# tangtang888/video-edge-ai-proxy

Measured on AMD Instinct MI355X. Metric: decoded FPS (whole node) + p50 VideoLatestImage latency, 256×1080p RTSP, higher is better.
Workload: dtype uint8 (BGR24 frames; bf16-capable consumer path)

## Files before the change

csrc/bind_ext.h:

```cpp
#pragma once
#include <pybind11/pybind11.h>

void bind_net(pybind11::module_& m);
void bind_mux(pybind11::module_& m);
void bind_hevc(pybind11::module_& m);
void bind_bus(pybind11::module_& m);
void bind_rpc(pybind11::module_& m);
void bind_dbk(pybind11::module_& m);
void bind_hevc_lf(pybind11::module_& m);
```

csrc/bindings.cpp:

```cpp
#include <malloc.h>

#include <pybind11/numpy.h>
#include <pybind11/pybind11.h>
#include <pybind11/stl.h>

#include "vep/hostprof.h"
#include "vep/avc.h"
#include "vep/avc_cavlc.h"
#include "vep/avc_recon.h"
#include "vep/bench_driver.h"
#include "vep/cabac.h"
#include "vep/codec.h"
#include "vep/gpu.h"
#include "vep/h264.h"
#include "vep/hevc_ctu.h"
#include "vep/hevc_dec.h"
#include "vep/hevc_kern.h"
#include "vep/jpeg.h"
#include "vep/scale.h"
#include "bind_ext.h"
#include "vep/runtime.h"
#include "vep/synth.h"

namespace py = pybind11;
// ... 2401 lines not shown
  m.def("letterbox_geometry", [](int src_w, int src_h, int size, bool even) {
    gpu::LetterboxDesc d{};
    d.src_w = src_w;
    d.src_h = src_h;
    gpu::fill_letterbox_geometry(d, size, even);
    return py::make_tuple(d.nw, d.nh, d.pad_x, d.pad_y);
  }, py::arg("src_w"), py::arg("src_h"), py::arg("size"), py::arg("even") = false);

  bind_net(m);
  bind_mux(m);
  bind_hevc(m);
  bind_bus(m);
  bind_rpc(m);
  bind_dbk(m);
  bind_hevc_lf(m);
}
```

csrc/vep/avc.cpp:

```cpp
#include "avc.h"

#include <immintrin.h>

#include <algorithm>
#include <array>

#include "avc_cavlc.h"
#include "avc_internal.h"
#include "fanout.h"

namespace vep::avc {

using h264::Pps;
using h264::Sps;


void MbNeighbours::reset(int wmbs, int hmbs, bool ring) {
  w_ = wmbs;
  h_ = hmbs;
  cur_ = -1;
  run_slice_ = ~0u;
  run_start_ = 0;
  announced_ = 0;
  const size_t n = size_t(wmbs) * hmbs;
// ... 1434 lines not shown
        }
        pair_.have |= u8(1 << int(sh.bottom_field));
        pair_.poc[int(sh.bottom_field)] = pic->poc;
      } else {
        pic->target = pick_slot();
      }
      if (sh.nal_ref_idc != 0 && sps.profile_idc != 66) {
        col_built = col_pool_->acquire([](ColMotion&) {});
        col_built->wmbs = W;
        col_built->hmbs = Hp;
        col_built->corners = sps.direct_8x8;
        col_built->b.resize(size_t(W) * Hp * size_t(sps.direct_8x8 ? 4 : 16));
        colb.col = col_built.get();
        pic->colb = &colb;
      }
      got = true;
    } else {
      VEP_CHECK(&sps == act_sps, "slices of one picture reference different SPSs");
      if (sh.field_pic != first.field_pic || sh.bottom_field != first.bottom_field) {
        VEP_CHECK(next_nal != nullptr, "H.264: one access unit holds several pictures");
        *next_nal = i;
        break;
      }
      if (sh.type() == h264::kB || pic->info.pict_type == 'I') pic->info.pict_type = "PBISi"[sh.type()];
    }
    if (sh.field_pic) build_field_lists(sh, sps, pic->poc);
    else build_lists(sh, sps, pic->poc);
    std::array<std::vector<u32>, 2> uids;
    for (int l = 0; l < 2; ++l)
      for (const auto& e : list_[l]) uids[size_t(l)].push_back(e.uid);
// ... 128 lines not shown
  } else {
    if (first.nal_ref_idc != 0) {
      mark_references(first, *act_sps, pic->target, pic->poc, uid, std::move(col_built));
    }
    const bool boundary = first.idr() || first.has_mmco5();
    if (first.has_mmco5()) pic->poc = 0;
    bump(*pic, out_of(*pic), boundary, boundary && (hard_flush || reorder_cur_ == 0));
  }
  if (missing || par) validate(*pic);
  else validate_picture(*pic);
  return pic;
}

Decoder::Decoder() {
  if (const char* e = std::getenv("VEP_AVC_SLICE_THREADS")) parallel_slices_ = e[0] != '0';
}
Decoder::~Decoder() = default;

void Decoder::parse_slice_data(MbNeighbours& nb, Picture& pic, const SliceHdr& sh, const Sps& sps, const Pps& pps,
                               const u8* data, size_t n, size_t bitpos, int slice_idx,
                               const std::vector<ListEntry> (&lists)[2]) {
  if (legacy_slice(sh, sps, pps)) {
    Bits br(data, n, bitpos);
    const size_t stop = BitReader(data, n).stop_bit_pos();
    SliceCtx sc{sh, pps, slice_idx, sh.type() == h264::kP, sh.qp, lists[0]};
    const int total = pic.nmbs();
    int mb = sh.first_mb;
    VEP_CHECK(mb < total, "first_mb_in_slice past end of picture");
    bool more = true;
    while (more) {
// ... 15 lines not shown
      more = br.pos() < stop;
      ++mb;
    }
    return;
  }
  SliceEnv env;
  env.sh = &sh;
  env.sps = &sps;
  env.pps = &pps;
  env.slice = slice_idx;
  env.list[0] = &lists[0];
  env.list[1] = &lists[1];
  env.cur_poc = pic.poc;
  env.scaling = h264::resolve_scaling(sps, pps);
  env.field = sh.field_pic;
  decode_slice_generic(nb, pic, env, data, n, bitpos);
}

static inline void validate_mb(const Picture& p, const MbRec& m, bool written = false) {
  const size_t ncoef = p.coefs.size(), nmv = p.mvs.size();
  VEP_CHECK(m.kind <= kI8x8, "macroblock kind out of range");
  VEP_CHECK(p.cf == 2 || m.chroma_coded < 0x100, "chroma block mask out of range");
  VEP_CHECK(m.qp <= 51 + p.qp_bias && m.qpc <= 51 + p.qpc_bias && m.qpc2 <= 51 + p.qpc_bias,
            "macroblock QP out of range");
  if (m.kind == kIPcm) {
    const size_t ns = p.cf == 2 ? size_t(kPcmMaxSamples) : size_t(kPcmMbBytes);
    VEP_CHECK(size_t(m.coef) + (p.bd > 8 ? ns : ns / 2) <= ncoef, "I_PCM samples outside the pool");
    return;
  }
  const size_t nw = size_t(coef_words(m));
// ... 354 lines not shown
  const __m256i tl = _mm256_setr_epi32(0, 0, 2, 2, 0, 0, 2, 2);
  const u32 all = u32(_mm256_movemask_epi8(_mm256_and_si256(_mm256_cmpeq_epi32(a, v0), _mm256_cmpeq_epi32(b, v0))));
  const u32 q8 = u32(_mm256_movemask_epi8(_mm256_and_si256(_mm256_cmpeq_epi32(a, _mm256_permutevar8x32_epi32(a, tl)),
                                                           _mm256_cmpeq_epi32(b, _mm256_permutevar8x32_epi32(b, tl)))));
  return (all == 0xFFFFFFFFu ? 1u : 0u) | (q8 == 0xFFFFFFFFu ? 2u : 0u);
#else
  u32 v[16];
  std::memcpy(v, mv, sizeof v);
  bool u16 = true, u8x8 = true;
  for (int b = 1; b < 16; ++b) u16 &= v[b] == v[0];
  for (int b = 0; b < 16; ++b) u8x8 &= v[b] == v[((b >> 3) << 3) | (b & 2)];
  return (u16 ? 1u : 0u) | (u8x8 ? 2u : 0u);
#endif
}

static inline void store_motion(Picture& pic, MbRec& m, const MbState& s) {
  const int nl = (m.flags & kMbL1) ? 2 : 1;
  u32 u = 3;
  for (int l = 0; l < nl; ++l) u &= motion_uniformity(&s.mv[l][0][0]);
  m.flags |= (u & 1) ? kMbMv16 : ((u & 2) ? kMbMv8x8 : 0);
  m.mv = u32(pic.mvs.size());
  const int per = (u & 1) ? 2 : ((u & 2) ? 8 : 32);
  i16* out = pic.mvs.extend(size_t(per * nl));
  for (int l = 0; l < nl; ++l, out += per) {
    const i16* v = &s.mv[l][0][0];
    if (per == 2) {
      std::memcpy(out, v, 4);
    } else if (per == 8) {
      std::memcpy(out, v, 4);
      std::memcpy(out + 2, v + 4, 4);
      std::memcpy(out + 4, v + 16, 4);
      std::memcpy(out + 6, v + 20, 4);
    } else {
      std::memcpy(out, v, 64);
// ... 15 lines not shown
  store_motion(pic, m, s);
  ++pic.inter_mbs;
  if (!(m.dbk & 1)) pic.deblock = true;
  for (int k = 0; k < 4; ++k) {
    const int r0 = m.ref[k], r1 = m.ref1[k];
    VEP_CHECK((r0 != 0xFF || r1 != 0xFF) && (r0 == 0xFF || r0 < pic.dpb_slots) && (r1 == 0xFF || r1 < pic.dpb_slots) &&
                  (r1 == 0xFF || (m.flags & kMbL1)),
              "skipped macroblock reference slot outside the DPB");
  }
  VEP_CHECK(m.qp <= 51 + pic.qp_bias && m.qpc <= 51 + pic.qpc_bias && m.qpc2 <= 51 + pic.qpc_bias,
            "macroblock QP out of range");
  store_rec(&pic.mbs[size_t(mb)], m);
  if (pic.colb) pic.colb->store(mb, s);
}

void store_mb(Picture& pic, int mb, MbRec m, const MbState& s, const MbResidual* res, const u8* pcm,
              const WpEntry* wp) {
  m.coef = u32(pic.coefs.size());
  m.luma_coded = 0;
  m.chroma_coded = 0;
  if (m.kind == kIPcm) {
    VEP_CHECK(pcm, "I_PCM macroblock without samples");
    const size_t ns = pic.cf == 2 ? size_t(kPcmMaxSamples) : size_t(kPcmMbBytes);
    const size_t o = pic.coefs.size(), nb = pic.bd > 8 ? 2 * ns : ns;
    pic.coefs.resize(o + nb / 2);
    std::memcpy(pic.coefs.data() + o, pcm, nb);
  } else if (res && (res->luma | res->chroma)) {
    m.luma_coded = res->luma;
    m.chroma_coded = res->chroma;
    if (res->t8) m.flags |= kMbT8x8;
    const i16* grp[32];
    int ng = 0;
// ... 10 lines not shown
    for (int g = 0; g < ng; ++g) {
      mask[g] = nonzero_mask16(grp[g]);
      nv += __builtin_popcount(mask[g]);
    }
    const size_t o = pic.coefs.size();
    i16* out = pic.coefs.extend(size_t(ng + nv) + 8);
    std::memcpy(out, mask, size_t(ng) * sizeof(u16));
    i16* v = out + ng;
    for (int g = 0; g < ng; ++g) v = compact16(grp[g], mask[g], v);
    pic.coefs.resize(o + size_t(ng + nv));
  }
  m.mv = 0;
  m.wp = 0;
  m.flags &= u8(~(kMbMv8x8 | kMbMv16));
  if (m.kind == kSkip || m.kind == kInter) {
    store_motion(pic, m, s);
    if (wp && (m.flags & kMbWp)) {
      m.wp = u32(pic.wps.size());
      pic.wps.insert(pic.wps.end(), wp, wp + 4);
    } else {
      m.flags &= u8(~kMbWp);
    }
    ++pic.inter_mbs;
  } else if (m.kind == kIPcm) {
    ++pic.inter_mbs;
  } else {
    ++pic.intra_mbs;
  }
  m.res = is_intra(m.kind) && m.kind != kIPcm && (m.luma_coded | m.chroma_coded) ? u32(pic.intra_res++) : kNoRes;
  if (!(m.dbk & 1)) pic.deblock = true;
  validate_written_mb(pic, m);
// ... 356 lines not shown
```

csrc/vep/avc.h:

```cpp
#pragma once

#include <array>
#include <map>
#include <memory>

#include "hostmem.h"
#include "recycle.h"
#include "avc_recon.h"
#include "codec.h"

namespace vep::avc {

constexpr int kMaxDpbSlots = 34;

struct AuMeta {
  i64 pts = 0, dts = 0, arrival_ms = 0;
  i64 tag = 0;
  bool keyframe = false, corrupt = false;
};

struct OutFrame {
  int slot = -1;
  PictureInfo info;
  AuMeta au;
// ... 71 lines not shown

struct MbState {
  u8 kind = 0xFF;
  u8 skip = 0;
  u8 direct16 = 0;
  u8 direct8 = 0;
  u8 t8x8 = 0;
  u8 cbp = 0;
  u8 chroma_mode = 0;
  u8 qp = 0;
  u16 slice = 0;
  u16 cbf = 0;
  u8 cbf_dc = 0;
  u8 cbf_cac[2] = {0, 0};
  i8 ref[2][4] = {{-1, -1, -1, -1}, {-1, -1, -1, -1}};
  i16 mv[2][16][2] = {};
  u8 mvd[2][16][2] = {};
  u8 tc[16] = {};
  u8 tcc[2][8] = {};
  u8 i4[16] = {};
};

class MbNeighbours {
 public:
  void reset(int wmbs, int hmbs, bool ring = false);
  void begin(int mb);
  MbState& at(int mb) { return st_[size_t(mb) & mask_]; }
  const MbState& at(int mb) const { return st_[size_t(mb) & mask_]; }
  int wmbs() const { return w_; }
  int hmbs() const { return h_; }
  int mb_at(int mb, int x, int y) const;
  bool mb_available(int mb, int nb) const {
    const size_t i = size_t(nb) & mask_;
    return nb >= 0 && stamp_[size_t(nb)] == epoch_ && tag_[i] == u32(nb) && st_[i].kind != 0xFF &&
           st_[i].slice == st_[size_t(mb) & mask_].slice;
// ... 320 lines not shown
  bool field_mode_ = false;
  struct OpenPair {
    bool open = false;
    int slot = -1, frame_num = 0, bottom = 0;
    int poc[2] = {0, 0};
    bool ref = false, boundary = false, hard = false;
    u8 have = 0;
    OutFrame f;
  } pair_;
  void close_pair(Picture& pic);

 public:
  Decoder();
  ~Decoder();
  u64 parallel_slices_run() const { return parallel_slices_run_; }
  u64 mmco_ops[7] = {0, 0, 0, 0, 0, 0, 0};
  u64 list_mods = 0, long_term_marked = 0;
  u64 redundant_slices_skipped = 0;
};

void cpu_reconstruct(const Picture& pic, std::vector<HostSurface>& slots);
void weave_fields(const HostSurface& top, const HostSurface& bottom, HostSurface& frame);

struct MbLevels {
  int luma[16][16];
  int dc[16];
  int cdc[2][4];
  int cac[2][4][16];
  u16 lmask = 0;
  u8 cmask = 0;
// ... 9 lines not shown
      for (int b = 0; b < 4; ++b) {
        if (cdc[c][b]) dcmask |= u8(2 << c);
        for (int k = 0; k < 16; ++k)
          if (cac[c][b][k]) cmask |= u8(1u << (c * 4 + b));
      }
  }
};
struct MbResidual {
  i16 blk[32][16];
  i16 b8[4][64];
  u16 luma = 0;
  u16 chroma = 0;
  bool t8 = false;
};
void dequantize_mb(const MbLevels& lv, bool i16x16, int qp, int qpc, MbResidual& out);
void store_mb(Picture& pic, int mb, MbRec m, const MbState& s, const MbResidual* res, const u8* pcm,
              const WpEntry* wp = nullptr);
void store_skip_mb(Picture& pic, int mb, MbRec& m, const MbState& s);
void cpu_reconstruct_mb(const Picture& pic, int mb, std::vector<HostSurface>& slots);
void cpu_deblock(const Picture& pic, HostSurface& target);
void intra4x4_neighbours(const Picture& pic, int mb, int idx, const HostSurface& T, Intra4Nb& n);
void intra16_neighbours(const Picture& pic, int mb, const HostSurface& T, Intra16Nb& n);
void chroma_neighbours(const Picture& pic, int mb, int c, const HostSurface& T, IntraChromaNb& n);
void intra8x8_neighbours(const Picture& pic, int mb, int q, const HostSurface& T, int* f, bool& has_top,
                         bool& has_left);

class StreamEncoder {
 public:
  virtual ~StreamEncoder() = default;
  virtual std::shared_ptr<AccessUnit> next() = 0;
  virtual const HostSurface& reconstruction() const = 0;
  virtual const HostSurface& source() const = 0;
  virtual i64 last_pts() const = 0;
// ... 93 lines not shown
```

csrc/vep/avc_internal.h:

```cpp
#pragma once

#include <array>

#include "avc.h"
#include "bits.h"

namespace vep::avc {

struct SliceEnv {
  const SliceHdr* sh = nullptr;
  const h264::Sps* sps = nullptr;
  const h264::Pps* pps = nullptr;
  int slice = 0;
  const std::vector<ListEntry>* list[2] = {nullptr, nullptr};
  int cur_poc = 0;
  h264::ScalingLists scaling;
  bool field = false;
};

void decode_slice_generic(MbNeighbours& nb, Picture& pic, const SliceEnv& env, const u8* data, size_t n,
                          size_t bitpos);

WpEntry wp_entry(const SliceEnv& env, int r0, int r1);

std::shared_ptr<ColMotion> build_col_motion(const MbNeighbours& nb, int wmbs, int hmbs,
                                            const std::vector<std::array<std::vector<u32>, 2>>& slice_uids,
                                            bool corners, Recycler<ColMotion>* pool = nullptr);

void predict_inter(const std::vector<HostSurface>& slots, const MbRec& m, const i16* mv0, const i16* mv1,
                   const WpEntry* wp, int mx, int my, int* py, int (*pc)[128], int structure = 0);

struct MbDesc {
// ... 54 lines not shown
```

csrc/vep/avc_mb.cpp:

```cpp
#include <algorithm>
#include <memory>
#include <cstddef>
#include <cstring>

#include "avc_cabac.h"
#include "avc_cavlc.h"
#include "avc_internal.h"

namespace vep::avc {

namespace {

struct Dequant {
  int ls4[6][6][16];
  int ls8[2][6][64];
  explicit Dequant(const h264::ScalingLists& sl) {
    for (int l = 0; l < 6; ++l)
      for (int m = 0; m < 6; ++m)
        for (int k = 0; k < 16; ++k) {
          const int pos = kZigzag4x4[k];
          ls4[l][m][pos] = int(sl.l4[l][k]) * norm_adjust(m, pos >> 2, pos & 3);
        }
    for (int l = 0; l < 2; ++l)
      for (int m = 0; m < 6; ++m)
// ... 48 lines not shown
    cf_ = sps_.chroma_format_idc;
    nbc_ = cf_ == 2 ? 8 : 4;
    weighted_ = (type_ == h264::kP && pps_.weighted_pred) || (type_ == h264::kB && pps_.weighted_bipred_idc != 0);
    implicit_ = type_ == h264::kB && pps_.weighted_bipred_idc == 2;
    for (int l = 0; l < 2; ++l) {
      std::fill(std::begin(slot_[l]), std::end(slot_[l]), u8(0xFF));
      if (const auto* lst = env_.list[l])
        for (size_t k = 0; k < lst->size() && k + 1 < std::size(slot_[l]); ++k)
          if ((*lst)[k].slot >= 0) slot_[l][k + 1] = u8((*lst)[k].slot);
    }
    for (int q = 0; q < 52 + qpbd_ && q < int(std::size(qpc_tab_[0])); ++q) {
      qpc_tab_[0][q] = u8(chroma_qp_bd(q - qpbd_, pps_.chroma_qp_index_offset, qpbdc_) + qpbdc_);
      qpc_tab_[1][q] = u8(chroma_qp_bd(q - qpbd_, pps_.second_chroma_qp_index_offset, qpbdc_) + qpbdc_);
    }
    fast_direct_ = !kWrite && type_ == h264::kB && sh_.direct_spatial && sps_.direct_8x8 && !weighted_;
  }

  Bits* br = nullptr;
  BitWriter* bw = nullptr;
  Bins* bins = nullptr;
  cabac::Decoder* cabac = nullptr;
  cabac::Encoder* cenc = nullptr;
  const MbDesc* want = nullptr;
  int prev_qpd_nz = 0;

  int qp() const { return qp_; }

  int ue(u32 v) {
    if constexpr (kWrite) {
      bw->ue(v);
      return int(v);
// ... 9 lines not shown
      return br->se();
    }
  }
  int u(int n, u32 v) {
    if constexpr (kWrite) {
      bw->u(n, v);
      return int(v);
    } else {
      return int(br->u(n));
    }
  }

  static void clear_but_mv(MbState& s) {
    static const MbState z{};
    std::memcpy(static_cast<void*>(&s), &z, offsetof(MbState, mv));
    std::memcpy(static_cast<void*>(&s.mvd), &z.mvd, sizeof(MbState) - offsetof(MbState, mvd));
  }

  bool read_skip_flag(int mb, bool v = false) {
    MbState& s = nb_.at(mb);
    if constexpr (kWrite) s = MbState{};
    else clear_but_mv(s);
    s.slice = u16(env_.slice);
    nb_.begin(mb);
    auto cond = [&](int m) { return m >= 0 && !nb_.at(m).skip ? 1 : 0; };
    const int inc = cond(nb_.mb_at(mb, -1, 0)) + cond(nb_.mb_at(mb, 0, -1));
    return bins->mb_skip(type_ == h264::kB, inc, v) != 0;
  }

  void skip_mb(int mb, bool fresh) {
    MbState& s = nb_.at(mb);
    if (fresh) {
      s = MbState{};
      s.slice = u16(env_.slice);
      nb_.begin(mb);
    }
    s.kind = kSkip;
    s.skip = 1;
    s.qp = u8(qp_ + qpbd_);
    MbResidual res;
    res.luma = 0;
    res.chroma = 0;
    if (type_ == h264::kP) {
      s.ref[0][0] = s.ref[0][1] = s.ref[0][2] = s.ref[0][3] = 0;
      need_ref(0, 0);
      int mv[2];
      nb_.pskip_mv(mb, mv);
      for (auto& v : s.mv[0]) {
        v[0] = i16(mv[0]);
        v[1] = i16(mv[1]);
      }
    } else {
      s.direct16 = 1;
      s.direct8 = 0xF;
      if (fast_direct_) direct16_spatial(mb, s);
      else direct(mb, s, 0xF);
    }
    prev_qpd_nz = 0;
    if (!weighted_ && !kWrite) emit_skip(mb, s);
    else emit(mb, s, res, 0, 0, nullptr);
  }

  void coded_mb(int mb, bool fresh) {
    MbState& s = nb_.at(mb);
    if (fresh) {
      s = MbState{};
      s.slice = u16(env_.slice);
      nb_.begin(mb);
    } else if constexpr (!kWrite) {
      std::memset(static_cast<void*>(s.mv), 0, sizeof s.mv);
    }
    int mbt = read_mb_type(mb, kWrite ? want->mb_type : 0);
    int itype = -1;
    if (type_ == h264::kI) {
      itype = mbt;
    } else if (type_ == h264::kP) {
      VEP_CHECK(mbt <= 30, "bad P mb_type");
      if (mbt >= 5) itype = mbt - 5;
    } else {
      VEP_CHECK(mbt <= 48, "bad B mb_type");
      if (mbt >= 23) itype = mbt - 23;
    }
    VEP_CHECK(itype <= 25, "bad intra mb_type");
    MbResidual res;
    res.luma = 0;
    res.chroma = 0;
// ... 26 lines not shown
    if (s.kind == kInter && (cbp & 15) && pps_.transform_8x8_mode && no_small &&
        !(type_ == h264::kB && mbt == 0 && !sps_.direct_8x8))
      s.t8x8 = u8(read_t8x8(mb, kWrite && want->t8x8));
    int qp = qp_;
    if ((cbp & 15) || (cbp >> 4) || s.kind == kI16x16) {
      const int dqp = read_qp_delta(kWrite ? want->qp_delta : 0);
      VEP_CHECK(dqp >= -(26 + qpbd_ / 2) && dqp <= 25 + qpbd_ / 2, "mb_qp_delta out of range");
      qp = (qp + dqp + 52 + 2 * qpbd_) % (52 + qpbd_) - qpbd_;
      prev_qpd_nz = dqp != 0;
    } else {
      prev_qpd_nz = 0;
    }
    qp_ = qp;
    s.qp = u8(qp + qpbd_);
    residual(mb, s, res, cbp & 15, cbp >> 4, qp + qpbd_, intra);
    emit(mb, s, res, i16_mode, s.chroma_mode, nullptr);
  }

  void skip_motion(int mb, MbState& out) {
    MbState& s = nb_.at(mb);
    s = MbState{};
    s.slice = u16(env_.slice);
    nb_.begin(mb);
    out = MbState{};
    out.slice = s.slice;
    if (type_ == h264::kP) {
      for (int k = 0; k < 4; ++k) out.ref[0][k] = 0;
      int mv[2];
      nb_.pskip_mv(mb, mv);
      for (auto& v : out.mv[0]) {
        v[0] = i16(mv[0]);
// ... 282 lines not shown
  }
  static void set_mv(MbState& s, int list, const Part& p, int mx, int my) {
    VEP_CHECK(mx >= -32768 && mx <= 32767 && my >= -32768 && my <= 32767, "motion vector out of range");
    for (int y = p.y4; y < p.y4 + p.h4; ++y)
      for (int x = p.x4; x < p.x4 + p.w4; ++x) {
        s.mv[list][y * 4 + x][0] = i16(mx);
        s.mv[list][y * 4 + x][1] = i16(my);
      }
  }

  bool inter_pred(int mb, MbState& s, int mbt) {
    const bool b = type_ == h264::kB;
    if (b && mbt == 0) {
      s.direct16 = 1;
      s.direct8 = 0xF;
      if (fast_direct_) direct16_spatial(mb, s);
      else direct(mb, s, 0xF);
      return true;
    }
    if ((!b && mbt <= 2) || (b && mbt <= 21)) {
      Part parts[2];
      int np;
      u8 pred[2];
      int shape;
      if (!b) {
        shape = mbt;
        pred[0] = pred[1] = 1;
      } else {
        shape = mbt <= 3 ? 0 : ((mbt & 1) ? 2 : 1);
        pred[0] = kBPart[mbt][0];
        pred[1] = kBPart[mbt][1];
      }
      np = shape == 0 ? 1 : 2;
      for (int i = 0; i < np; ++i) {
        if (shape == 0) parts[i] = {0, 0, 4, 4, 0};
        else if (shape == 1) parts[i] = {0, 2 * i, 4, 2, 1};
        else parts[i] = {2 * i, 0, 2, 4, 2};
      }
      int refs[2][2] = {{-1, -1}, {-1, -1}};
      for (int l = 0; l < 2; ++l)
        for (int i = 0; i < np; ++i) {
          if (!((pred[i] >> l) & 1)) continue;
          refs[l][i] = read_ref(mb, l, parts[i].x4, parts[i].y4, kWrite ? want->ref[l][i] : 0);
          const Part& p = parts[i];
          for (int y = p.y4 / 2; y < (p.y4 + p.h4) / 2; ++y)
            for (int x = p.x4 / 2; x < (p.x4 + p.w4) / 2; ++x) s.ref[l][y * 2 + x] = i8(refs[l][i]);
        }
      int mvd[2][2][2] = {};
// ... 101 lines not shown
        done[1] |= b8_blocks(i);
      }
    };
    if constexpr (kWrite) derive(true);
    for (int l = 0; l < 2; ++l)
      for (int i = 0; i < 4; ++i) {
        if (!((spred[i] >> l) & 1)) continue;
        for (int j = 0; j < kSubParts[sshape[i]]; ++j) {
          const Part p = sub_part(i, j);
          mvd[l][i][j][0] = read_mvd(mb, l, p.x4, p.y4, 0, mvd[l][i][j][0]);
          mvd[l][i][j][1] = read_mvd(mb, l, p.x4, p.y4, 1, mvd[l][i][j][1]);
          set_mvd(s, l, p, mvd[l][i][j][0], mvd[l][i][j][1]);
        }
      }
    if constexpr (!kWrite) derive(false);
    return no_small;
  }

  void direct(int mb, MbState& s, int mask) {
    VEP_CHECK(env_.list[1] && !env_.list[1]->empty() && (*env_.list[1])[0].slot >= 0,
              "direct prediction without a list-1 reference");
    const ListEntry& c1 = (*env_.list[1])[0];
    const ColMotion* col = c1.col;
    VEP_CHECK(col && col->wmbs == nb_.wmbs() && col->hmbs == nb_.hmbs() && col->corners == sps_.direct_8x8,
              "colocated picture motion missing");
    const bool infer = sps_.direct_8x8;
    auto fill = [&](int l, int b8, int blk, int mx, int my) {
      if (!infer) {
        s.mv[l][blk][0] = i16(mx);
        s.mv[l][blk][1] = i16(my);
// ... 58 lines not shown
          const int tx = (16384 + std::abs(td / 2)) / td;
          const int dsf = clip3i(-1024, 1023, (tb * tx + 32) >> 6);
          for (int k = 0; k < 2; ++k) {
            m0[k] = (dsf * mvc[k] + 128) >> 8;
            m1[k] = m0[k] - mvc[k];
          }
        }
        fill(0, b8, blk, clip3i(-32768, 32767, m0[0]), clip3i(-32768, 32767, m0[1]));
        fill(1, b8, blk, clip3i(-32768, 32767, m1[0]), clip3i(-32768, 32767, m1[1]));
      }
      s.ref[0][b8] = i8(r0);
      s.ref[1][b8] = 0;
    }
  }

  void direct16_spatial(int mb, MbState& s) {
    if (!dcol_) {
      VEP_CHECK(env_.list[1] && !env_.list[1]->empty() && (*env_.list[1])[0].slot >= 0,
                "direct prediction without a list-1 reference");
      const ListEntry& c1 = (*env_.list[1])[0];
      VEP_CHECK(c1.col && c1.col->wmbs == nb_.wmbs() && c1.col->hmbs == nb_.hmbs() && c1.col->corners,
                "colocated picture motion missing");
      dcol_ = c1.col;
      dcol_long_ = c1.long_term;
    }
    int ref[2], mvp[2][2];
    nb_.direct_spatial_both(ref, mvp);
    const bool zero = ref[0] < 0 && ref[1] < 0;
    if (zero) ref[0] = ref[1] = 0;
    u32 pv[2];
    for (int l = 0; l < 2; ++l) {
// ... 6 lines not shown
    u32 v8[2][4];
    for (int b8 = 0; b8 < 4; ++b8) {
      const bool col_zero = !dcol_long_ && cb[b8].ref == 0 && cb[b8].mv[0] >= -1 && cb[b8].mv[0] <= 1 &&
                            cb[b8].mv[1] >= -1 && cb[b8].mv[1] <= 1;
      for (int l = 0; l < 2; ++l) v8[l][b8] = (ref[l] == 0 && col_zero) ? 0u : pv[l];
    }
    for (int l = 0; l < 2; ++l) {
      u32 row[2][4];
      for (int h = 0; h < 2; ++h) {
        row[h][0] = row[h][1] = v8[l][2 * h];
        row[h][2] = row[h][3] = v8[l][2 * h + 1];
      }
      u8* mv = reinterpret_cast<u8*>(&s.mv[l][0][0]);
      for (int y = 0; y < 4; ++y) std::memcpy(mv + 16 * y, row[y >> 1], 16);
    }
  }

  WpEntry weights(int r0, int r1) { return wp_entry(env_, r0, r1); }

  int cbf_luma_inc(int mb, int blk, bool intra) {
    auto cond = [&](int m, int nblk) -> int {
      if (m < 0) return intra ? 1 : 0;
      const MbState& n = nb_.at(m);
      if (n.kind == kIPcm) return 1;
      if (n.skip) return 0;
      if (!((n.cbp >> raster_b8(nblk)) & 1)) return 0;
      if (n.t8x8) return 1;
      return (n.cbf >> nblk) & 1;
    };
    const int bx = blk & 3, by = blk >> 2;
// ... 193 lines not shown
            for (int j = 0; j < tc; ++j) {
              const int k = nzp[j];
              const int pos = scan4_[k + 1];
              const int v = scale4(lv[k], dq_.ls4[lc][qpc[c] % 6][pos], qpc[c]);
              d[pos] = sat16(v);
              nz |= v != 0;
            }
          }
          if (nz) res.chroma |= u16(1u << (c * nbc + b));
        }
      }
    }
    if constexpr (!kCabac && !kWrite) VEP_CHECK(!br->overrun(), "slice data overrun");
  }

  void emit(int mb, const MbState& s, const MbResidual& res, int i16_mode, int chroma_mode, const u8* pcm) {
    MbRec m{};
    m.kind = s.kind;
    m.qp = u8(s.kind == kIPcm ? qpbd_ : s.qp);
    VEP_CHECK(m.qp < std::size(qpc_tab_[0]), "macroblock QP out of range");
    m.qpc = qpc_tab_[0][m.qp];
    m.qpc2 = qpc_tab_[1][m.qp];
    m.i16_mode = u8(i16_mode);
    m.chroma_mode = u8(chroma_mode);
    m.dbk = u8((sh_.disable_deblocking == 1 ? 1 : 0) | (sh_.disable_deblocking == 2 ? 2 : 0));
    m.alpha_off = i8(sh_.alpha_off);
    m.beta_off = i8(sh_.beta_off);
    m.slice = s.slice;
    m.flags = s.t8x8 && s.kind != kI8x8 ? kMbT8x8 : 0;
    if (s.kind == kI8x8) m.flags = kMbT8x8;
    bool l1 = false;
// ... 22 lines not shown
      for (int r = 0; r < 16; ++r) m.i4[r >> 1] |= u8(s.i4[r] << ((r & 1) * 4));
    if (s.kind == kI8x8)
      for (int b8 = 0; b8 < 4; ++b8) m.i4[b8 >> 1] |= u8(s.i4[(b8 & 1) * 2 + (b8 >> 1) * 8] << ((b8 & 1) * 4));
    WpEntry wp[4];
    bool use_wp = false;
    if (weighted_ && !is_intra(s.kind)) {
      for (int k = 0; k < 4; ++k) {
        wp[k] = weights(s.ref[0][k], s.ref[1][k]);
        const WpEntry& e = wp[k];
        for (int c = 0; c < 3; ++c)
          use_wp |= !(e.lwd[c] == 0 && e.w0[c] == 1 && e.w1[c] == 1 && e.o[c] == 0) &&
                    !(e.w0[c] == (1 << e.lwd[c]) && e.w1[c] == (1 << e.lwd[c]) && e.o[c] == 0);
      }
      if (use_wp) m.flags |= kMbWp;
    }
    store_mb(pic_, mb, m, s, &res, pcm, use_wp ? wp : nullptr);
  }

  void emit_skip(int mb, const MbState& s) {
    MbRec m{};
    m.kind = kSkip;
    m.qp = s.qp;
    VEP_CHECK(m.qp < std::size(qpc_tab_[0]), "macroblock QP out of range");
    m.qpc = qpc_tab_[0][m.qp];
    m.qpc2 = qpc_tab_[1][m.qp];
    m.dbk = u8((sh_.disable_deblocking == 1 ? 1 : 0) | (sh_.disable_deblocking == 2 ? 2 : 0));
    m.alpha_off = i8(sh_.alpha_off);
    m.beta_off = i8(sh_.beta_off);
    m.slice = s.slice;
    bool l1 = false;
    for (int k = 0; k < 4; ++k) {
      m.ref[k] = slot_[0][s.ref[0][k] + 1];
      m.ref1[k] = slot_[1][s.ref[1][k] + 1];
      l1 |= s.ref[1][k] >= 0;
    }
    m.flags = l1 ? kMbL1 : 0;
    nz8_ = 0;
    store_skip_mb(pic_, mb, m, s);
  }

  MbNeighbours& nb_;
  Picture& pic_;
  const SliceEnv& env_;
  const SliceHdr& sh_;
  const h264::Pps& pps_;
  const h264::Sps& sps_;
  const Dequant& dq_;
  const u8* scan4_;
  const u8* scan8_;
  int type_ = 0;
  int qp_ = 26;
  bool weighted_ = false, implicit_ = false;
  u16 nz8_ = 0;
  u8 slot_[2][33];
  u8 qpc_tab_[2][96];
  bool fast_direct_ = false;
  const ColMotion* dcol_ = nullptr;
  bool dcol_long_ = false;
};

}

WpEntry wp_entry(const SliceEnv& env, int r0, int r1) {
  const SliceHdr& sh = *env.sh;
  const bool implicit = sh.type() == h264::kB && env.pps->weighted_bipred_idc == 2;
  WpEntry e{};
  for (int c = 0; c < 3; ++c) {
    e.w0[c] = e.w1[c] = 1;
    e.o[c] = 0;
    e.lwd[c] = 0;
  }
  if (implicit) {
    if (r0 < 0 || r1 < 0) return e;
// ... 54 lines not shown
      throw UnsupportedStream("CABAC cabac_init_idc " + std::to_string(sh.cabac_init_idc) + " is not supported");
    const size_t start = (bitpos + 7) >> 3;
    VEP_CHECK(start <= n, "slice data overrun");
    cabac::Ctx ctx[kCabacCtx];
    cabac_init_contexts(ctx, sh.type() == h264::kI ? -1 : 0, std::max(0, sh.qp));
    cabac::Decoder dec(data, n, start);
    BinDecoder bd{dec, ctx};
    AvcBins<BinDecoder> bins{bd};
    MbLayer<true, false> L(nb, pic, env, dq);
    L.bins = &bins;
    L.cabac = &dec;
    L.data = data;
    L.data_n = n;
    for (;;) {
      VEP_CHECK(mb < total, "macroblock address past end of picture");
      if (sh.type() != h264::kI && L.read_skip_flag(mb)) L.skip_mb(mb, false);
      else L.coded_mb(mb, sh.type() == h264::kI);
      ++mb;
      if (bins.end_of_slice(false)) {
        cabac::bins_decoded().fetch_add(dec.bins(), std::memory_order_relaxed);
        break;
      }
      VEP_CHECK(dec.bitpos() <= n * 8 + 16, "slice data overrun");
    }
    return;
  }
  Bits br(data, n, bitpos);
  const size_t stop = BitReader(data, n).stop_bit_pos();
  MbLayer<false, false> L(nb, pic, env, dq);
  L.br = &br;
  bool more = true;
  while (more) {
// ... 98 lines not shown
```

csrc/vep/cabac.h:

```cpp
#pragma once

#include <atomic>
#include <cstring>

#include "common.h"

namespace vep::cabac {

#define VEP_CABAC_INLINE inline __attribute__((always_inline))

inline constexpr u8 kRangeLps[64][4] = {
    {128, 176, 208, 240}, {128, 167, 197, 227}, {128, 158, 187, 216}, {123, 150, 178, 205},
    {116, 142, 169, 195}, {111, 135, 160, 185}, {105, 128, 152, 175}, {100, 122, 144, 166},
    {95, 116, 137, 158},  {90, 110, 130, 150},  {85, 104, 123, 142},  {81, 99, 117, 135},
    {77, 94, 111, 128},   {73, 89, 105, 122},   {69, 85, 100, 116},   {66, 80, 95, 110},
    {62, 76, 90, 104},    {59, 72, 86, 99},     {56, 69, 81, 94},     {53, 65, 77, 89},
    {51, 62, 73, 85},     {48, 59, 69, 80},     {46, 56, 66, 76},     {43, 53, 63, 72},
    {41, 50, 59, 69},     {39, 48, 56, 65},     {37, 45, 54, 62},     {35, 43, 51, 59},
    {33, 41, 48, 56},     {32, 39, 46, 53},     {30, 37, 43, 50},     {29, 35, 41, 48},
    {27, 33, 39, 45},     {26, 31, 37, 43},     {24, 30, 35, 41},     {23, 28, 33, 39},
    {22, 27, 32, 37},     {21, 26, 30, 35},     {20, 24, 29, 33},     {19, 23, 27, 31},
    {18, 22, 26, 30},     {17, 21, 25, 28},     {16, 20, 23, 27},     {15, 19, 22, 25},
    {14, 18, 21, 24},     {14, 17, 20, 23},     {13, 16, 19, 22},     {12, 15, 18, 21},
    {12, 14, 17, 20},     {11, 14, 16, 19},     {11, 13, 15, 18},     {10, 12, 15, 17},
// ... 69 lines not shown
  }
  VEP_CABAC_INLINE u32 decision(Ctx& c) {
    ++nbins_;
    const u64 e = c.e;
    const u32 lps = Ctx::lps_of(e, range_);
    u64 e_lps = kCtxWords.e[(e >> 40) & 127], e_mps = kCtxWords.e[(e >> 48) & 127];
    asm("" : "+r"(e_lps), "+r"(e_mps));
    const u32 rmps = range_ - lps;
    const u32 is_lps = offset_ >= rmps ? 1u : 0u;
    offset_ -= rmps & (0u - is_lps);
    range_ = is_lps ? lps : rmps;
    c.e = is_lps ? e_lps : e_mps;
    renorm();
    return (u32(e >> 32) & 1u) ^ is_lps;
  }
  u32 terminate() {
    ++nbins_;
    range_ -= 2;
    if (offset_ >= range_) return 1;
    renorm();
    return 0;
  }
  VEP_CABAC_INLINE u32 bypass() {
    ++nbins_;
    offset_ = (offset_ << 1) | bits(1);
    const u32 b = offset_ >= range_ ? 1u : 0u;
    offset_ -= range_ & (0u - b);
    return b;
  }
  size_t bitpos() const { return byte_ * 8 - size_t(cbits_); }
  u64 bins() const { return nbins_; }
// ... 171 lines not shown
```

Baseline: 8422.

## Add fast CABAC skip-run path with templated skip MB records and motion granularity hints

Adds a fast path for CABAC P/B slices that decodes runs of skip flags in a tight loop using a local copy of the CABAC decoder. Skip macroblocks are written from a precomputed MbRec template with non-temporal stores. Known motion granularity (16x16 or 8x8) is passed through to store_motion so it can skip the generic uniformity scan. MbState is reordered so clearing touches fewer bytes, and a new Python binding dumps parsed pools for verification. Risks include subtle mismatches in neighbour state or skip context handling, and streaming stores evicting data that is read again soon.

```diff
diff --git a/csrc/bind_avc_parse.cpp b/csrc/bind_avc_parse.cpp
--- /dev/null
+++ b/csrc/bind_avc_parse.cpp
@@ -0,0 +1,84 @@
+#include <pybind11/pybind11.h>
+#include <pybind11/stl.h>
+
+#include <cstring>
+#include <string>
+#include <vector>
+
+#include "bind_ext.h"
+#include "vep/avc.h"
+#include "vep/cabac.h"
+#include "vep/codec.h"
+
+namespace py = pybind11;
+using namespace vep;
+
+namespace {
+
+template <class T>
+void put(std::string& out, const T& v) {
+  out.append(reinterpret_cast<const char*>(&v), sizeof v);
+}
+
+struct ParsedPools {
+  std::string mbs, mvs, coefs, wps, col;
+  char type = '?';
+};
+
+}
+
+void bind_avc_parse(py::module_& m) {
+  m.def(
+      "avc_parse_pools",
+      [](const std::vector<std::shared_ptr<AccessUnit>>& aus, bool fast) {
+        std::vector<ParsedPools> pics;
+        u64 bins = 0;
+        {
+          py::gil_scoped_release r;
+          avc::Decoder dec;
+          dec.set_mb_fast(fast);
+          dec.keep_last_col = true;
+          const u64 bins0 = cabac::bins_decoded().load();
+          for (const auto& au : aus) {
+            size_t nal = 0;
+            do {
+              avc::PicturePtr p = dec.parse(*au, 0, &nal);
+              if (!p) continue;
+              static_assert(sizeof(avc::MbRec) == 56, "MbRec has no implicit padding");
+              ParsedPools o;
+              o.type = p->info.pict_type;
+              o.mbs.assign(reinterpret_cast<const char*>(p->mbs.data()), p->mbs.size() * sizeof(avc::MbRec));
+              o.mvs.assign(reinterpret_cast<const char*>(p->mvs.data()), p->mvs.size() * sizeof(i16));
+              o.coefs.assign(reinterpret_cast<const char*>(p->coefs.data()), p->coefs.size() * sizeof(i16));
+              o.wps.assign(reinterpret_cast<const char*>(p->wps.data()), p->wps.size() * sizeof(avc::WpEntry));
+              if (auto col = dec.last_col()) {
+                put(o.col, col->wmbs);
+                put(o.col, col->hmbs);
+                put(o.col, u8(col->corners));
+                for (const avc::ColMotion::Blk& b : col->b) {
+                  put(o.col, b.mv[0]);
+                  put(o.col, b.mv[1]);
+                  put(o.col, b.pid);
+                  put(o.col, b.ref);
+                }
+              }
+              pics.push_back(std::move(o));
+            } while (nal < au->nals.size());
+          }
+          bins = cabac::bins_decoded().load() - bins0;
+        }
+        py::list out;
+        for (const ParsedPools& o : pics) {
+          py::dict d;
+          d["type"] = std::string(1, o.type);
+          d["mbs"] = py::bytes(o.mbs);
+          d["mvs"] = py::bytes(o.mvs);
+          d["coefs"] = py::bytes(o.coefs);
+          d["wps"] = py::bytes(o.wps);
+          d["col"] = py::bytes(o.col);
+          out.append(d);
+        }
+        return py::make_tuple(out, bins);
+      },
+      py::arg("aus"), py::arg("fast") = true);
+}
diff --git a/csrc/bind_ext.h b/csrc/bind_ext.h
--- a/csrc/bind_ext.h
+++ b/csrc/bind_ext.h
@@ -8,3 +8,4 @@
 void bind_rpc(pybind11::module_& m);
 void bind_dbk(pybind11::module_& m);
 void bind_hevc_lf(pybind11::module_& m);
+void bind_avc_parse(pybind11::module_& m);
diff --git a/csrc/bindings.cpp b/csrc/bindings.cpp
--- a/csrc/bindings.cpp
+++ b/csrc/bindings.cpp
@@ -2439,4 +2439,5 @@
   bind_rpc(m);
   bind_dbk(m);
   bind_hevc_lf(m);
+  bind_avc_parse(m);
 }
diff --git a/csrc/vep/avc.cpp b/csrc/vep/avc.cpp
--- a/csrc/vep/avc.cpp
+++ b/csrc/vep/avc.cpp
@@ -4,6 +4,7 @@
 
 #include <algorithm>
 #include <array>
+#include <cstddef>
 
 #include "avc_cavlc.h"
 #include "avc_internal.h"
@@ -1472,6 +1473,7 @@
         colb.col = col_built.get();
         pic->colb = &colb;
       }
+      if (keep_last_col) last_col_ = col_built;
       got = true;
     } else {
       VEP_CHECK(&sps == act_sps, "slices of one picture reference different SPSs");
@@ -1630,6 +1632,7 @@
 
 Decoder::Decoder() {
   if (const char* e = std::getenv("VEP_AVC_SLICE_THREADS")) parallel_slices_ = e[0] != '0';
+  if (const char* e = std::getenv("VEP_AVC_MB_FAST")) mb_fast_ = e[0] != '0';
 }
 Decoder::~Decoder() = default;
 
@@ -1675,6 +1678,7 @@
   env.cur_poc = pic.poc;
   env.scaling = h264::resolve_scaling(sps, pps);
   env.field = sh.field_pic;
+  env.fast = mb_fast_;
   decode_slice_generic(nb, pic, env, data, n, bitpos);
 }
 
@@ -2059,10 +2063,25 @@
 #endif
 }
 
-static inline void store_motion(Picture& pic, MbRec& m, const MbState& s) {
+static inline void store_motion(Picture& pic, MbRec& m, const MbState& s, int gran = kMotionUnknown) {
   const int nl = (m.flags & kMbL1) ? 2 : 1;
   u32 u = 3;
-  for (int l = 0; l < nl; ++l) u &= motion_uniformity(&s.mv[l][0][0]);
+  if (gran == kMotion16) {
+    u = 3;
+  } else if (gran == kMotion8x8) {
+    bool same = true;
+    for (int l = 0; l < nl; ++l) {
+      u32 v0, v1, v2, v3;
+      std::memcpy(&v0, &s.mv[l][0][0], 4);
+      std::memcpy(&v1, &s.mv[l][2][0], 4);
+      std::memcpy(&v2, &s.mv[l][8][0], 4);
+      std::memcpy(&v3, &s.mv[l][10][0], 4);
+      same &= (v0 == v1) & (v0 == v2) & (v0 == v3);
+    }
+    u = same ? 3 : 2;
+  } else {
+    for (int l = 0; l < nl; ++l) u &= motion_uniformity(&s.mv[l][0][0]);
+  }
   m.flags |= (u & 1) ? kMbMv16 : ((u & 2) ? kMbMv8x8 : 0);
   m.mv = u32(pic.mvs.size());
   const int per = (u & 1) ? 2 : ((u & 2) ? 8 : 32);
@@ -2108,8 +2127,48 @@
   if (pic.colb) pic.colb->store(mb, s);
 }
 
+void store_skip_tpl(Picture& pic, int mb, const MbRec& tpl, u32 ref0, u32 ref1, bool l1, int gran, const MbState& s) {
+  const int nl = l1 ? 2 : 1, per = gran == kMotion16 ? 2 : 8;
+  const u32 mvo = u32(pic.mvs.size()), coef = u32(pic.coefs.size());
+  i16* out = pic.mvs.extend(size_t(per * nl));
+  for (int l = 0; l < nl; ++l, out += per) {
+    const i16* v = &s.mv[l][0][0];
+    std::memcpy(out, v, 4);
+    if (per == 8) {
+      std::memcpy(out + 2, v + 4, 4);
+      std::memcpy(out + 4, v + 16, 4);
+      std::memcpy(out + 6, v + 20, 4);
+    }
+  }
+  ++pic.inter_mbs;
+  if (!(tpl.dbk & 1)) pic.deblock = true;
+  const u8 flags = u8((l1 ? kMbL1 : 0) | (gran == kMotion16 ? kMbMv16 : kMbMv8x8));
+#if defined(__x86_64__)
+  static_assert(offsetof(MbRec, flags) == 7 && offsetof(MbRec, ref) == 20 && offsetof(MbRec, ref1) == 24 &&
+                    offsetof(MbRec, coef) == 28 && offsetof(MbRec, mv) == 32 && offsetof(MbRec, i4) == 36,
+                "MbRec words");
+  u64 w[7];
+  std::memcpy(w, &tpl, sizeof w);
+  w[0] |= u64(flags) << 56;
+  w[2] |= u64(ref0) << 32;
+  w[3] = u64(ref1) | u64(coef) << 32;
+  w[4] = u64(mvo);
+  long long* d = reinterpret_cast<long long*>(&pic.mbs[size_t(mb)]);
+  for (int k = 0; k < 7; ++k) _mm_stream_si64(d + k, static_cast<long long>(w[k]));
+#else
+  MbRec m = tpl;
+  m.flags = flags;
+  std::memcpy(m.ref, &ref0, 4);
+  std::memcpy(m.ref1, &ref1, 4);
+  m.coef = coef;
+  m.mv = mvo;
+  store_rec(&pic.mbs[size_t(mb)], m);
+#endif
+  if (pic.colb) pic.colb->store(mb, s);
+}
+
 void store_mb(Picture& pic, int mb, MbRec m, const MbState& s, const MbResidual* res, const u8* pcm,
-              const WpEntry* wp) {
+              const WpEntry* wp, int gran) {
   m.coef = u32(pic.coefs.size());
   m.luma_coded = 0;
   m.chroma_coded = 0;
@@ -2150,7 +2209,7 @@
   m.wp = 0;
   m.flags &= u8(~(kMbMv8x8 | kMbMv16));
   if (m.kind == kSkip || m.kind == kInter) {
-    store_motion(pic, m, s);
+    store_motion(pic, m, s, gran);
     if (wp && (m.flags & kMbWp)) {
       m.wp = u32(pic.wps.size());
       pic.wps.insert(pic.wps.end(), wp, wp + 4);
diff --git a/csrc/vep/avc.h b/csrc/vep/avc.h
--- a/csrc/vep/avc.h
+++ b/csrc/vep/avc.h
@@ -109,11 +109,11 @@
   u8 cbf_dc = 0;
   u8 cbf_cac[2] = {0, 0};
   i8 ref[2][4] = {{-1, -1, -1, -1}, {-1, -1, -1, -1}};
-  i16 mv[2][16][2] = {};
   u8 mvd[2][16][2] = {};
   u8 tc[16] = {};
   u8 tcc[2][8] = {};
   u8 i4[16] = {};
+  i16 mv[2][16][2] = {};
 };
 
 class MbNeighbours {
@@ -464,6 +464,16 @@
   Decoder();
   ~Decoder();
   u64 parallel_slices_run() const { return parallel_slices_run_; }
+  bool mb_fast() const { return mb_fast_; }
+  void set_mb_fast(bool on) { mb_fast_ = on; }
+  bool keep_last_col = false;
+  std::shared_ptr<const ColMotion> last_col() const { return last_col_; }
+
+ private:
+  bool mb_fast_ = true;
+  std::shared_ptr<const ColMotion> last_col_;
+
+ public:
   u64 mmco_ops[7] = {0, 0, 0, 0, 0, 0, 0};
   u64 list_mods = 0, long_term_marked = 0;
   u64 redundant_slices_skipped = 0;
@@ -503,9 +513,13 @@
   bool t8 = false;
 };
 void dequantize_mb(const MbLevels& lv, bool i16x16, int qp, int qpc, MbResidual& out);
+constexpr int kMotionUnknown = 0;
+constexpr int kMotion16 = 1;
+constexpr int kMotion8x8 = 2;
 void store_mb(Picture& pic, int mb, MbRec m, const MbState& s, const MbResidual* res, const u8* pcm,
-              const WpEntry* wp = nullptr);
+              const WpEntry* wp = nullptr, int gran = kMotionUnknown);
 void store_skip_mb(Picture& pic, int mb, MbRec& m, const MbState& s);
+void store_skip_tpl(Picture& pic, int mb, const MbRec& tpl, u32 ref0, u32 ref1, bool l1, int gran, const MbState& s);
 void cpu_reconstruct_mb(const Picture& pic, int mb, std::vector<HostSurface>& slots);
 void cpu_deblock(const Picture& pic, HostSurface& target);
 void intra4x4_neighbours(const Picture& pic, int mb, int idx, const HostSurface& T, Intra4Nb& n);
diff --git a/csrc/vep/avc_internal.h b/csrc/vep/avc_internal.h
--- a/csrc/vep/avc_internal.h
+++ b/csrc/vep/avc_internal.h
@@ -16,6 +16,7 @@
   int cur_poc = 0;
   h264::ScalingLists scaling;
   bool field = false;
+  bool fast = true;
 };
 
 void decode_slice_generic(MbNeighbours& nb, Picture& pic, const SliceEnv& env, const u8* data, size_t n,
diff --git a/csrc/vep/avc_mb.cpp b/csrc/vep/avc_mb.cpp
--- a/csrc/vep/avc_mb.cpp
+++ b/csrc/vep/avc_mb.cpp
@@ -86,7 +86,20 @@
       qpc_tab_[1][q] = u8(chroma_qp_bd(q - qpbd_, pps_.second_chroma_qp_index_offset, qpbdc_) + qpbdc_);
     }
     fast_direct_ = !kWrite && type_ == h264::kB && sh_.direct_spatial && sps_.direct_8x8 && !weighted_;
-  }
+    fast_ = !kWrite && env.fast;
+    tpl_ = MbRec{};
+    tpl_.kind = kSkip;
+    tpl_.dbk = u8((sh_.disable_deblocking == 1 ? 1 : 0) | (sh_.disable_deblocking == 2 ? 2 : 0));
+    tpl_.alpha_off = i8(sh_.alpha_off);
+    tpl_.beta_off = i8(sh_.beta_off);
+    tpl_.slice = u16(env_.slice);
+    tpl_.res = kNoRes;
+    tpl_ok_ = fast_ && !weighted_;
+    for (int l = 0; l < 2; ++l)
+      for (u8 sl : slot_[l]) tpl_ok_ &= sl == 0xFF || sl < pic_.dpb_slots;
+  }
+
+  bool fast() const { return fast_; }
 
   Bits* br = nullptr;
   BitWriter* bw = nullptr;
@@ -126,7 +139,10 @@
   static void clear_but_mv(MbState& s) {
     static const MbState z{};
     std::memcpy(static_cast<void*>(&s), &z, offsetof(MbState, mv));
-    std::memcpy(static_cast<void*>(&s.mvd), &z.mvd, sizeof(MbState) - offsetof(MbState, mvd));
+  }
+  static void clear_head(MbState& s) {
+    static const MbState z{};
+    std::memcpy(static_cast<void*>(&s), &z, offsetof(MbState, i4));
   }
 
   bool read_skip_flag(int mb, bool v = false) {
@@ -140,6 +156,33 @@
     return bins->mb_skip(type_ == h264::kB, inc, v) != 0;
   }
 
+  int skip_run(int mb, int total, bool& ended) {
+    ended = false;
+    if constexpr (kCabac && !kWrite) {
+      cabac::Ctx* const ctx = bins->e.ctx + (type_ == h264::kB ? 24 : 11);
+      cabac::Decoder d = *cabac;
+      for (;;) {
+        VEP_CHECK(mb < total, "macroblock address past end of picture");
+        MbState& s = nb_.at(mb);
+        clear_head(s);
+        s.slice = u16(env_.slice);
+        nb_.begin(mb);
+        const int am = nb_.mb_at(mb, -1, 0), bm = nb_.mb_at(mb, 0, -1);
+        const int inc = (am >= 0 && !nb_.at(am).skip ? 1 : 0) + (bm >= 0 && !nb_.at(bm).skip ? 1 : 0);
+        if (!d.decision(ctx[inc])) break;
+        skip_body(mb, s);
+        ++mb;
+        if (d.terminate()) {
+          ended = true;
+          break;
+        }
+        VEP_CHECK(d.bitpos() <= data_n * 8 + 16, "slice data overrun");
+      }
+      *cabac = d;
+    }
+    return mb;
+  }
+
   void skip_mb(int mb, bool fresh) {
     MbState& s = nb_.at(mb);
     if (fresh) {
@@ -147,6 +190,11 @@
       s.slice = u16(env_.slice);
       nb_.begin(mb);
     }
+    skip_body(mb, s);
+  }
+
+  void skip_body(int mb, MbState& s) {
+    int gran = kMotionUnknown;
     s.kind = kSkip;
     s.skip = 1;
     s.qp = u8(qp_ + qpbd_);
@@ -162,15 +210,17 @@
         v[0] = i16(mv[0]);
         v[1] = i16(mv[1]);
       }
+      gran = kMotion16;
     } else {
       s.direct16 = 1;
       s.direct8 = 0xF;
-      if (fast_direct_) direct16_spatial(mb, s);
+      if (fast_direct_) gran = direct16_spatial(mb, s);
       else direct(mb, s, 0xF);
     }
     prev_qpd_nz = 0;
-    if (!weighted_ && !kWrite) emit_skip(mb, s);
-    else emit(mb, s, res, 0, 0, nullptr);
+    if (tpl_ok_ && gran != kMotionUnknown) emit_skip_tpl(mb, s, gran);
+    else if (!weighted_ && !kWrite) emit_skip(mb, s);
+    else emit(mb, s, res, 0, 0, nullptr, fast_ ? gran : kMotionUnknown);
   }
 
   void coded_mb(int mb, bool fresh) {
@@ -182,6 +232,7 @@
     } else if constexpr (!kWrite) {
       std::memset(static_cast<void*>(s.mv), 0, sizeof s.mv);
     }
+    gran_ = kMotionUnknown;
     int mbt = read_mb_type(mb, kWrite ? want->mb_type : 0);
     int itype = -1;
     if (type_ == h264::kI) {
@@ -238,7 +289,7 @@
     qp_ = qp;
     s.qp = u8(qp + qpbd_);
     residual(mb, s, res, cbp & 15, cbp >> 4, qp + qpbd_, intra);
-    emit(mb, s, res, i16_mode, s.chroma_mode, nullptr);
+    emit(mb, s, res, i16_mode, s.chroma_mode, nullptr, fast_ ? gran_ : kMotionUnknown);
   }
 
   void skip_motion(int mb, MbState& out) {
@@ -551,7 +602,7 @@
     if (b && mbt == 0) {
       s.direct16 = 1;
       s.direct8 = 0xF;
-      if (fast_direct_) direct16_spatial(mb, s);
+      if (fast_direct_) gran_ = direct16_spatial(mb, s);
       else direct(mb, s, 0xF);
       return true;
     }
@@ -569,6 +620,7 @@
         pred[1] = kBPart[mbt][1];
       }
       np = shape == 0 ? 1 : 2;
+      gran_ = shape == 0 ? kMotion16 : kMotion8x8;
       for (int i = 0; i < np; ++i) {
         if (shape == 0) parts[i] = {0, 0, 4, 4, 0};
         else if (shape == 1) parts[i] = {0, 2 * i, 4, 2, 1};
@@ -700,6 +752,7 @@
         }
       }
     if constexpr (!kWrite) derive(false);
+    if (no_small) gran_ = kMotion8x8;
     return no_small;
   }
 
@@ -788,7 +841,7 @@
     }
   }
 
-  void direct16_spatial(int mb, MbState& s) {
+  int direct16_spatial(int mb, MbState& s) {
     if (!dcol_) {
       VEP_CHECK(env_.list[1] && !env_.list[1]->empty() && (*env_.list[1])[0].slot >= 0,
                 "direct prediction without a list-1 reference");
@@ -825,6 +878,9 @@
       u8* mv = reinterpret_cast<u8*>(&s.mv[l][0][0]);
       for (int y = 0; y < 4; ++y) std::memcpy(mv + 16 * y, row[y >> 1], 16);
     }
+    bool same = true;
+    for (int l = 0; l < 2; ++l) same &= (v8[l][0] == v8[l][1]) & (v8[l][0] == v8[l][2]) & (v8[l][0] == v8[l][3]);
+    return same ? kMotion16 : kMotion8x8;
   }
 
   WpEntry weights(int r0, int r1) { return wp_entry(env_, r0, r1); }
@@ -1048,7 +1104,8 @@
     if constexpr (!kCabac && !kWrite) VEP_CHECK(!br->overrun(), "slice data overrun");
   }
 
-  void emit(int mb, const MbState& s, const MbResidual& res, int i16_mode, int chroma_mode, const u8* pcm) {
+  void emit(int mb, const MbState& s, const MbResidual& res, int i16_mode, int chroma_mode, const u8* pcm,
+            int gran = kMotionUnknown) {
     MbRec m{};
     m.kind = s.kind;
     m.qp = u8(s.kind == kIPcm ? qpbd_ : s.qp);
@@ -1101,7 +1158,7 @@
       }
       if (use_wp) m.flags |= kMbWp;
     }
-    store_mb(pic_, mb, m, s, &res, pcm, use_wp ? wp : nullptr);
+    store_mb(pic_, mb, m, s, &res, pcm, use_wp ? wp : nullptr, gran);
   }
 
   void emit_skip(int mb, const MbState& s) {
@@ -1124,6 +1181,22 @@
     m.flags = l1 ? kMbL1 : 0;
     nz8_ = 0;
     store_skip_mb(pic_, mb, m, s);
+  }
+
+  void emit_skip_tpl(int mb, const MbState& s, int gran) {
+    if (s.qp != tpl_qp_) tpl_set_qp(s.qp);
+    const u32 r0 = 0x01010101u * slot_[0][s.ref[0][0] + 1], r1 = 0x01010101u * slot_[1][s.ref[1][0] + 1];
+    nz8_ = 0;
+    store_skip_tpl(pic_, mb, tpl_, r0, r1, s.ref[1][0] >= 0, gran, s);
+  }
+  void tpl_set_qp(int qp) {
+    VEP_CHECK(size_t(qp) < std::size(qpc_tab_[0]), "macroblock QP out of range");
+    tpl_.qp = u8(qp);
+    tpl_.qpc = qpc_tab_[0][qp];
+    tpl_.qpc2 = qpc_tab_[1][qp];
+    VEP_CHECK(tpl_.qp <= 51 + pic_.qp_bias && tpl_.qpc <= 51 + pic_.qpc_bias && tpl_.qpc2 <= 51 + pic_.qpc_bias,
+              "macroblock QP out of range");
+    tpl_qp_ = qp;
   }
 
   MbNeighbours& nb_;
@@ -1144,6 +1217,11 @@
   bool fast_direct_ = false;
   const ColMotion* dcol_ = nullptr;
   bool dcol_long_ = false;
+  bool fast_ = false;
+  bool tpl_ok_ = false;
+  MbRec tpl_{};
+  int tpl_qp_ = -1;
+  int gran_ = kMotionUnknown;
 };
 
 }
@@ -1228,8 +1306,19 @@
     L.data_n = n;
     for (;;) {
       VEP_CHECK(mb < total, "macroblock address past end of picture");
-      if (sh.type() != h264::kI && L.read_skip_flag(mb)) L.skip_mb(mb, false);
-      else L.coded_mb(mb, sh.type() == h264::kI);
+      if (sh.type() != h264::kI && L.fast()) {
+        bool ended;
+        mb = L.skip_run(mb, total, ended);
+        if (ended) {
+          cabac::bins_decoded().fetch_add(dec.bins(), std::memory_order_relaxed);
+          break;
+        }
+        L.coded_mb(mb, false);
+      } else if (sh.type() != h264::kI && L.read_skip_flag(mb)) {
+        L.skip_mb(mb, false);
+      } else {
+        L.coded_mb(mb, sh.type() == h264::kI);
+      }
       ++mb;
       if (bins.end_of_slice(false)) {
         cabac::bins_decoded().fetch_add(dec.bins(), std::memory_order_relaxed);
diff --git a/csrc/vep/cabac.h b/csrc/vep/cabac.h
--- a/csrc/vep/cabac.h
+++ b/csrc/vep/cabac.h
@@ -107,7 +107,7 @@
     renorm();
     return (u32(e >> 32) & 1u) ^ is_lps;
   }
-  u32 terminate() {
+  VEP_CABAC_INLINE u32 terminate() {
     ++nbins_;
     range_ -= 2;
     if (offset_ >= range_) return 1;
```

After: 8331. 0.989x the previous value.
